# Zehong-Ma/MagCache

Measured on NVIDIA H100. Metric: denoising_steps_per_sec, higher is better.
Workload: dtype bf16

## Files before the change

magcache_b200/build.py:

```python
import os
import shutil
import subprocess
import sys

HERE = os.path.dirname(os.path.abspath(__file__))
CSRC = os.path.join(HERE, "csrc")
LIB = os.path.join(HERE, "libmagcache_b200.so")
SOURCES = ["controller.cu", "cache_kernels.cu", "rowwise_kernels.cu", "gemm_wgmma.cu", "attn_wgmma.cu", "head_wgmma.cu", "p2p.cu", "dit_forward.cu", "nccl_gather.cu"]
NVCC_FLAGS = ["-gencode", "arch=compute_90a,code=sm_90a", "-O3", "-std=c++17", "-lineinfo", "-Xcompiler", "-fPIC",
              "-Xptxas", "-v", "--expt-relaxed-constexpr"]


def _nvcc():
    return shutil.which("nvcc") or "/usr/local/cuda/bin/nvcc"


def _stale():
    if not os.path.exists(LIB):
        return True
    t = os.path.getmtime(LIB)
    deps = [os.path.join(CSRC, f) for f in os.listdir(CSRC)] + [os.path.join(HERE, "..", "include", "magcache_b200.h"), __file__]
    return any(os.path.getmtime(d) > t for d in deps)


def build(force=False, verbose=False):
    if not force and not _stale():
        return LIB
    objs = []
    bdir = os.path.join(HERE, "build")
    os.makedirs(bdir, exist_ok=True)
    procs = []
    for src in SOURCES:
        obj = os.path.join(bdir, src.replace(".cu", ".o"))
        cmd = [_nvcc(), *NVCC_FLAGS, "-c", os.path.join(CSRC, src), "-o", obj]
        procs.append((src, subprocess.Popen(cmd, stdout=subprocess.PIPE, stderr=subprocess.STDOUT, text=True)))
        objs.append(obj)
    log = []
    for src, p in procs:
        out, _ = p.communicate()
        log.append(f"==== {src}\n{out}")
        if p.returncode != 0:
            sys.stderr.write(out)
            raise RuntimeError(f"nvcc failed on {src}")
    with open(os.path.join(bdir, "ptxas.log"), "w") as f:
        f.write("\n".join(log))
    if verbose:
        print("\n".join(log))
    serialised = [line.strip() for line in "\n".join(log).splitlines() if "C7510" in line]
    if serialised:
        raise RuntimeError("ptxas serialised wgmma (C7510); no kernel that issues wgmma may contain a function call such as "
                           "device printf (see MC_DEVICE_DIAG in csrc/ptx.cuh). Full log: build/ptxas.log\n" +
                           "\n".join(serialised[:8]))
    cmd = [_nvcc(), "-shared", "-o", LIB, *objs, "-gencode", "arch=compute_90a,code=sm_90a", "-cudart", "static", "-ldl"]
    subprocess.check_call(cmd)
    return LIB


if __name__ == "__main__":
    print(build(force="--force" in sys.argv, verbose="-v" in sys.argv))
```

magcache_b200/csrc/attn_wgmma.cu:

```cuda
#include <cstdlib>

#include "common.cuh"
#include "ptx.cuh"
#include "tma_host.cuh"

#ifndef MC_ATTN_EMU_DEFAULT
#define MC_ATTN_EMU_DEFAULT 0
#endif

namespace mc {

constexpr int kHD = 128;
constexpr int kLongMinLk = 1024;

struct AttnParams {
  int Lq, Lk, heads;
  int q_blocks, full_units, tail_units, tail_split;
  float* part_o;
  float2* part_ml;
  float scale_log2;
  __nv_bfloat16* out;
  int64_t ldo;
  int tile_rot;
  const uint32_t* seg_flags;
// ... 13 lines not shown
  if (c < p.full_units) {
    unit = c, w.split = 0, w.nsplit = 1, w.tail_unit = 0;
  } else {
    c -= p.full_units;
    w.tail_unit = c / p.tail_split;
    w.split = c - w.tail_unit * p.tail_split;
    w.nsplit = p.tail_split;
    unit = p.full_units + w.tail_unit;
  }
  w.head = unit / p.q_blocks;
  w.q_block = unit - w.head * p.q_blocks;
  return w;
}

template <uint32_t EMU_MASK>
__device__ __forceinline__ float exp2_sel(float x, int group) {
  return ((EMU_MASK >> (group & 7)) & 1u) ? ptx::ex2_emul(x) : ptx::ex2_approx(x);
}

__device__ __forceinline__ void wait_segments(const AttnParams& p, int row0, int rows) {
  if (p.seg_flags == nullptr) return;
  const uint32_t want = *reinterpret_cast<const volatile uint32_t*>(p.seg_epoch);
  const int last = min(row0 + rows, p.Lk) - 1;
  const int s0 = row0 / p.seg_rows, s1 = last / p.seg_rows;
  for (int s = s0; s <= s1; ++s) {
    const uint32_t* f = p.seg_flags + s;
    const long long t0 = clock64();
    for (;;) {
      uint32_t v;
      asm volatile("ld.acquire.sys.global.u32 %0, [%1];" : "=r"(v) : "l"(f) : "memory");
      if (static_cast<int32_t>(v - want) >= 0) break;
      __nanosleep(100);
      if (clock64() - t0 > MC_MBAR_TIMEOUT_CYCLES) {
        MC_DIAG("attention: key segment %d never arrived (flag %u, epoch %u)\n", s, v, want);
        __trap();
      }
    }
  }
  asm volatile("fence.proxy.async;" ::: "memory");
}

namespace ak {
constexpr int kBQ = 128;
constexpr int kQBytes = kBQ * kHD * 2;
constexpr int kThreads = 384;
constexpr int kProducerRegs = 24, kConsumerRegs = 240;
template <int BKV>
struct Layout {
  static constexpr int kKBytes = BKV * kHD * 2;
  static constexpr int kVBytes = BKV * kHD * 2;
  static constexpr int kOffK = kQBytes;
  static constexpr int kOffV = kOffK + 2 * kKBytes;
  static constexpr int kOffBar = kOffV + 2 * kVBytes;
  static constexpr int kSmem = kOffBar + 128;
};
}

template <int BKV, uint32_t EMU_MASK>
__global__ void __launch_bounds__(ak::kThreads, 1)
    attn_kernel(const __grid_constant__ CUtensorMap tmap_q, const __grid_constant__ CUtensorMap tmap_k,
                const __grid_constant__ CUtensorMap tmap_v, const AttnParams p) {
  using namespace ak;
  using L = Layout<BKV>;
  extern __shared__ __align__(1024) uint8_t smem[];
  uint64_t* bars = reinterpret_cast<uint64_t*>(smem + L::kOffBar);
  uint64_t* q_full = bars + 0;
  uint64_t* k_full = bars + 1;
  uint64_t* k_empty = bars + 3;
  uint64_t* v_full = bars + 5;
  uint64_t* v_empty = bars + 7;

  const int warp = threadIdx.x >> 5, lane = threadIdx.x & 31;
  const WorkItem wi = work_item(p);
  const int q0 = wi.q_block * kBQ;
  const int head = wi.head;
  const int total_tiles = (p.Lk + BKV - 1) / BKV;
  const int per_split = (total_tiles + wi.nsplit - 1) / wi.nsplit;
  const int t0 = wi.split * per_split;
  const int n_tiles = min(per_split, total_tiles - t0);
  auto tile_of = [&](int j) {
    int t = p.tile_rot + t0 + j;
    return t >= total_tiles ? t - total_tiles : t;
  };

  if (threadIdx.x == 0) {
    if ((ptx::smem_u32(smem) & 1023u) != 0) {
      MC_DIAG("attn_kernel: dynamic smem base not 1024-aligned\n");
      __trap();
    }
    ptx::prefetch_tmap(&tmap_q);
    ptx::prefetch_tmap(&tmap_k);
    ptx::prefetch_tmap(&tmap_v);
    ptx::mbar_init(q_full, 1);
    for (int s = 0; s < 2; ++s) {
      ptx::mbar_init(&k_full[s], 1);
      ptx::mbar_init(&k_empty[s], 8);
      ptx::mbar_init(&v_full[s], 1);
      ptx::mbar_init(&v_empty[s], 8);
    }
    ptx::fence_mbar_init();
  }
  __syncthreads();

  if (warp < 4) {
    ptx::setmaxnreg_dec<kProducerRegs>();
    if (warp == 0) {
      if (ptx::elect_one()) {
        ptx::mbar_expect_tx(q_full, kQBytes);
        ptx::tma_load_2d(smem, &tmap_q, q_full, head * kHD, q0);
        ptx::tma_load_2d(smem + kQBytes / 2, &tmap_q, q_full, head * kHD + 64, q0);
      }
      __syncwarp();
      for (int j = 0; j < n_tiles; ++j) {
        const int s = j & 1;
        const uint32_t ph = (j >> 1) & 1;
        const int kv0 = tile_of(j) * BKV;
        if (p.seg_flags != nullptr) {
          if (lane == 0) wait_segments(p, kv0, BKV);
          __syncwarp();
        }
        ptx::mbar_wait(&k_empty[s], ph ^ 1);
        if (ptx::elect_one()) {
          ptx::mbar_expect_tx(&k_full[s], L::kKBytes);
          ptx::tma_load_2d(smem + L::kOffK + s * L::kKBytes, &tmap_k, &k_full[s], head * kHD, kv0);
          ptx::tma_load_2d(smem + L::kOffK + s * L::kKBytes + L::kKBytes / 2, &tmap_k, &k_full[s], head * kHD + 64, kv0);
        }
        __syncwarp();
        ptx::mbar_wait(&v_empty[s], ph ^ 1);
        if (ptx::elect_one()) {
          ptx::mbar_expect_tx(&v_full[s], L::kVBytes);
          ptx::tma_load_2d(smem + L::kOffV + s * L::kVBytes, &tmap_v, &v_full[s], head * kHD, kv0);
          ptx::tma_load_2d(smem + L::kOffV + s * L::kVBytes + L::kVBytes / 2, &tmap_v, &v_full[s], head * kHD + 64, kv0);
        }
        __syncwarp();
      }
    }
  } else {
    ptx::setmaxnreg_inc<kConsumerRegs>();
    const int wg = (warp >> 2) - 1;
    const int r = wg * 64 + (warp & 3) * 16 + (lane >> 2);
    const int cq = 2 * (lane & 3);
    const uint32_t q_base = ptx::smem_u32(smem) + wg * (64 * 128);
    const uint32_t k_base = ptx::smem_u32(smem + L::kOffK), v_base = ptx::smem_u32(smem + L::kOffV);
    int j_ragged = -1;
    if (p.Lk % BKV != 0) {
      int jr = total_tiles - 1 - p.tile_rot - t0;
      if (jr < 0) jr += total_tiles;
      if (jr < n_tiles) j_ragged = jr;
    }
    float o[kHD / 2];
#pragma unroll
    for (int i = 0; i < kHD / 2; ++i) o[i] = 0.f;
    float m0 = -INFINITY, m1 = -INFINITY, l0 = 0.f, l1 = 0.f;
    ptx::mbar_wait(q_full, 0);

    constexpr uint32_t kTurnThreads = 256;
    const uint32_t bar_own = 1 + wg, bar_other = 2 - wg;
    auto turn_begin = [&] { ptx::named_bar_sync(bar_own, kTurnThreads); };
    auto turn_end = [&] { ptx::named_bar_arrive(bar_other, kTurnThreads); };
    if (wg == 0) ptx::named_bar_arrive(bar_own, kTurnThreads);

    float sc[BKV / 2];
    uint32_t pa[BKV / 16][4];
    const int valid = p.Lk - (total_tiles - 1) * BKV;
    auto issue_s = [&](int j) {
      const int s = j & 1;
      ptx::wgmma_fence();
#pragma unroll
      for (int kk = 0; kk < kHD / 16; ++kk) {
        const uint64_t da = ptx::gmma_desc_sw128_kmajor(q_base + (kk >> 2) * (kQBytes / 2)) + 2 * (kk & 3);
        const uint64_t db = ptx::gmma_desc_sw128_kmajor(k_base + s * L::kKBytes + (kk >> 2) * (L::kKBytes / 2)) + 2 * (kk & 3);
        if constexpr (BKV == 128) {
          ptx::wgmma_m64n128k16_ss(sc, da, db, kk != 0 ? 1u : 0u);
        } else {
          ptx::wgmma_m64n64k16_ss(sc, da, db, kk != 0 ? 1u : 0u);
        }
      }
      ptx::wgmma_commit();
    };
    auto issue_pv = [&](int j) {
      const int s = j & 1;
      ptx::fence_regs(o);
      ptx::wgmma_fence();
      const uint64_t dv = ptx::gmma_desc_sw128_mnmajor(v_base + s * L::kVBytes, BKV * 128);
#pragma unroll
      for (int kk = 0; kk < BKV / 16; ++kk)
        ptx::wgmma_m64n128k16_rs_tb(o, pa[kk], dv + static_cast<uint64_t>(kk * (2048 / 16)), 1u);
      ptx::wgmma_commit();
    };
    auto softmax = [&](int j, float& f0, float& f1) {
      ptx::fence_regs(sc);
      __syncwarp();
      if (lane == 0) ptx::mbar_arrive(&k_empty[j & 1]);
      if (j == j_ragged) {
#pragma unroll
        for (int i = 0; i < BKV / 8; ++i)
#pragma unroll
          for (int e = 0; e < 4; ++e)
            if (8 * i + cq + (e & 1) >= valid) sc[4 * i + e] = -INFINITY;
      }
      float mx0 = -INFINITY, mx1 = -INFINITY;
#pragma unroll
      for (int i = 0; i < BKV / 8; ++i) {
        mx0 = fmaxf(mx0, fmaxf(sc[4 * i], sc[4 * i + 1]));
        mx1 = fmaxf(mx1, fmaxf(sc[4 * i + 2], sc[4 * i + 3]));
      }
#pragma unroll
      for (int off = 1; off <= 2; off <<= 1) {
        mx0 = fmaxf(mx0, __shfl_xor_sync(0xffffffffu, mx0, off));
        mx1 = fmaxf(mx1, __shfl_xor_sync(0xffffffffu, mx1, off));
      }
      const float mn0 = fmaxf(m0, mx0 * p.scale_log2), mn1 = fmaxf(m1, mx1 * p.scale_log2);
      f0 = ptx::ex2_approx(m0 - mn0), f1 = ptx::ex2_approx(m1 - mn1);
      m0 = mn0, m1 = mn1;
      l0 *= f0, l1 *= f1;
#pragma unroll
      for (int i = 0; i < BKV / 8; ++i) {
        sc[4 * i] = exp2_sel<EMU_MASK>(fmaf(sc[4 * i], p.scale_log2, -m0), i);
        sc[4 * i + 1] = exp2_sel<EMU_MASK>(fmaf(sc[4 * i + 1], p.scale_log2, -m0), i);
        sc[4 * i + 2] = exp2_sel<EMU_MASK>(fmaf(sc[4 * i + 2], p.scale_log2, -m1), i);
        sc[4 * i + 3] = exp2_sel<EMU_MASK>(fmaf(sc[4 * i + 3], p.scale_log2, -m1), i);
        l0 += sc[4 * i] + sc[4 * i + 1];
        l1 += sc[4 * i + 2] + sc[4 * i + 3];
      }
    };
    auto pack_p = [&] {
#pragma unroll
      for (int i = 0; i < BKV / 8; ++i) {
        pa[i >> 1][(i & 1) * 2] = pack_bf16x2(sc[4 * i], sc[4 * i + 1]);
        pa[i >> 1][(i & 1) * 2 + 1] = pack_bf16x2(sc[4 * i + 2], sc[4 * i + 3]);
      }
    };
    auto release_v = [&](int j) {
      ptx::fence_regs(o);
      __syncwarp();
      if (lane == 0) ptx::mbar_arrive(&v_empty[j & 1]);
    };
    auto rescale_o = [&](float f0, float f1) {
#pragma unroll
      for (int i = 0; i < kHD / 8; ++i) {
        o[4 * i] *= f0, o[4 * i + 1] *= f0;
        o[4 * i + 2] *= f1, o[4 * i + 3] *= f1;
      }
    };
    for (int j = 0; j < n_tiles; ++j) {
      ptx::mbar_wait(&k_full[j & 1], (j >> 1) & 1);
      turn_begin();
      issue_s(j);
      turn_end();
      ptx::wgmma_wait<0>();
      float f0, f1;
      softmax(j, f0, f1);
      rescale_o(f0, f1);
      pack_p();
      ptx::mbar_wait(&v_full[j & 1], (j >> 1) & 1);
      turn_begin();
      issue_pv(j);
      if (wg == 0 || j + 1 < n_tiles) turn_end();
      ptx::wgmma_wait<0>();
      release_v(j);
    }

#pragma unroll
    for (int off = 1; off <= 2; off <<= 1) {
      l0 += __shfl_xor_sync(0xffffffffu, l0, off);
      l1 += __shfl_xor_sync(0xffffffffu, l1, off);
    }
    const bool partial = wi.nsplit > 1;
#pragma unroll
    for (int h = 0; h < 2; ++h) {
      const float inv_l = 1.0f / (h ? l1 : l0);
      const int rt = r + 8 * h;
      const int row = q0 + rt;
      if (row >= p.Lq) continue;
      if (partial) {
        const int64_t prow = (static_cast<int64_t>(wi.split) * p.tail_units + wi.tail_unit) * kBQ + rt;
        if ((lane & 3) == 0) p.part_ml[prow] = make_float2(h ? m1 : m0, h ? l1 : l0);
        float* dst = p.part_o + prow * kHD + cq;
#pragma unroll
        for (int i = 0; i < kHD / 8; ++i)
          *reinterpret_cast<float2*>(dst + 8 * i) = make_float2(o[4 * i + 2 * h] * inv_l, o[4 * i + 2 * h + 1] * inv_l);
      } else {
        __nv_bfloat16* dst = p.out + static_cast<int64_t>(row) * p.ldo + head * kHD + cq;
#pragma unroll
        for (int i = 0; i < kHD / 8; ++i)
          *reinterpret_cast<uint32_t*>(dst + 8 * i) = pack_bf16x2(o[4 * i + 2 * h] * inv_l, o[4 * i + 2 * h + 1] * inv_l);
      }
    }
  }
}

__global__ void __launch_bounds__(256) attn_combine_kernel(const float* __restrict__ part_o, const float2* __restrict__ part_ml, int nsplit,
                                                           int tail_units, int full_units, int q_blocks, int rows_per_cta, int Lq,
                                                           __nv_bfloat16* __restrict__ out, int64_t ldo) {
  constexpr int kGroups = kHD / 8;
  const int64_t total = static_cast<int64_t>(tail_units) * rows_per_cta * kGroups;
  const int64_t split_stride = static_cast<int64_t>(tail_units) * rows_per_cta;
  for (int64_t i = static_cast<int64_t>(blockIdx.x) * blockDim.x + threadIdx.x; i < total; i += static_cast<int64_t>(gridDim.x) * blockDim.x) {
    const int64_t prow = i / kGroups;
    const int g = static_cast<int>(i - prow * kGroups);
    const int tu = static_cast<int>(prow / rows_per_cta), r = static_cast<int>(prow - static_cast<int64_t>(tu) * rows_per_cta);
    const int unit = full_units + tu;
    const int head = unit / q_blocks, row = (unit - head * q_blocks) * rows_per_cta + r;
    if (row >= Lq) continue;
    float mmax = -INFINITY;
    for (int s = 0; s < nsplit; ++s) mmax = fmaxf(mmax, part_ml[s * split_stride + prow].x);
    float acc[8] = {0.f, 0.f, 0.f, 0.f, 0.f, 0.f, 0.f, 0.f};
    float wsum = 0.f;
    for (int s = 0; s < nsplit; ++s) {
      const float2 ml = part_ml[s * split_stride + prow];
      const float w = ml.y * ptx::ex2_approx(ml.x - mmax);
      wsum += w;
      float v[8];
      ptx::ld_nc_v8_f32(part_o + (s * split_stride + prow) * kHD + g * 8, v);
#pragma unroll
      for (int j = 0; j < 8; ++j) acc[j] = fmaf(w, v[j], acc[j]);
    }
    const float inv = 1.0f / wsum;
#pragma unroll
    for (int j = 0; j < 8; ++j) acc[j] *= inv;
    *reinterpret_cast<uint4*>(out + static_cast<int64_t>(row) * ldo + head * kHD + g * 8) = pack_bf16x8(acc);
  }
}

struct AttnPlan {
  bool long_kernel;
  int q_blocks, kv_tile, total_tiles, rows_per_cta;
  int full_units, tail_units, tail_split;
  size_t ws_bytes;
  int grid() const { return full_units + tail_units * tail_split; }
};

static int env_int(const char* name, int lo, int hi, int dflt) {
  const char* e = getenv(name);
  if (!e || !*e) return dflt;
  const int v = atoi(e);
  return (v < lo || v > hi) ? dflt : v;
}

static AttnPlan plan_attention(int Lq, int Lk, int heads, bool need_long = false) {
  AttnPlan pl;
  const int forced_splits = env_int("MC_ATTN_SPLITS", 1, 16, 0);
  const int kernel_sel = env_int("MC_ATTN_KERNEL", 0, 2, 0);
  pl.long_kernel = need_long || kernel_sel == 2 || (kernel_sel == 0 && Lk >= kLongMinLk);
  pl.rows_per_cta = ak::kBQ;
  pl.kv_tile = pl.long_kernel ? 128 : 64;
  pl.q_blocks = (Lq + pl.rows_per_cta - 1) / pl.rows_per_cta;
  pl.total_tiles = (Lk + pl.kv_tile - 1) / pl.kv_tile;
  const int64_t units = static_cast<int64_t>(pl.q_blocks) * heads;
  const int slots = num_sms();
  const int min_tiles_per_split = pl.long_kernel ? 4 : 8;
  int full = static_cast<int>(units), tail = 0, split = 1;
  if (forced_splits > 0) {
    if (forced_splits > 1) full = 0, tail = static_cast<int>(units), split = forced_splits;
  } else {
    const int rem = static_cast<int>(units % slots);
    const int by_tiles = pl.total_tiles / min_tiles_per_split;
    int f = rem > 0 ? slots / rem : 1;
    if (f > 8) f = 8;
    if (f > by_tiles) f = by_tiles;
    if (f >= 2) full = static_cast<int>(units) - rem, tail = rem, split = f;
  }
  if (split > pl.total_tiles) split = pl.total_tiles;
  if (split > 1) {
    const int per = (pl.total_tiles + split - 1) / split;
    split = (pl.total_tiles + per - 1) / per;
  }
  if (split <= 1) full = static_cast<int>(units), tail = 0, split = 1;
  pl.full_units = full, pl.tail_units = tail, pl.tail_split = split;
  pl.ws_bytes = tail > 0 ? static_cast<size_t>(split) * tail * pl.rows_per_cta * (kHD * sizeof(float) + sizeof(float2)) : 0;
  return pl;
}

}

extern "C" int32_t mc_attn_workspace_bytes(int32_t Lq, int32_t Lk, int32_t heads, int64_t* bytes_out) {
  MC_CHECK_ARG(bytes_out != nullptr && Lq >= 1 && Lk >= 1 && heads >= 1, "mc_attn_workspace_bytes: bad arguments");
  const size_t a = mc::plan_attention(Lq, Lk, heads, false).ws_bytes, b = mc::plan_attention(Lq, Lk, heads, true).ws_bytes;
  *bytes_out = static_cast<int64_t>(a > b ? a : b);
  return MC_OK;
}

extern "C" int32_t mc_attn_fwd_ex(const void* q, int64_t ldq, const void* k, int64_t ldk, const void* v, int64_t ldv, void* out,
                                  int64_t ldo, int32_t Lq, int32_t Lk, int32_t heads, float scale, void* workspace,
                                  int64_t workspace_bytes, int32_t first_key_row, const uint32_t* seg_flags, const uint32_t* seg_epoch,
                                  int32_t seg_rows, void* stream) {
  MC_CHECK_ARG(q && k && v && out, "mc_attn_fwd: null pointer");
  MC_CHECK_ARG(Lq >= 1 && Lk >= 1 && heads >= 1, "mc_attn_fwd: Lq=%d Lk=%d heads=%d", Lq, Lk, heads);
  const int64_t width = static_cast<int64_t>(heads) * mc::kHD;
  MC_CHECK_ARG(ldq >= width && ldk >= width && ldo >= width && ldv >= width, "mc_attn_fwd: leading dimensions too small");
  MC_CHECK_ARG(ldq % 8 == 0 && ldk % 8 == 0 && ldv % 8 == 0 && ldo % 8 == 0, "mc_attn_fwd: leading dimensions must be multiples of 8");
  MC_CHECK_ARG(mc::aligned16(q) && mc::aligned16(k) && mc::aligned16(v) && mc::aligned16(out), "mc_attn_fwd: pointers must be 16-byte aligned");
  MC_CHECK_ARG(first_key_row >= 0 && first_key_row < Lk, "mc_attn_fwd: first_key_row=%d outside [0, %d)", first_key_row, Lk);
  MC_CHECK_ARG(seg_flags == nullptr || (seg_rows >= 1 && seg_epoch != nullptr), "mc_attn_fwd: seg_rows=%d / null epoch", seg_rows);
  const mc::AttnPlan pl = mc::plan_attention(Lq, Lk, heads, first_key_row != 0 || seg_flags != nullptr);
  MC_CHECK_ARG(static_cast<int64_t>(pl.q_blocks) * heads * 8 < INT32_MAX, "mc_attn_fwd: grid too large");
  if (pl.tail_units > 0) {
    MC_CHECK_ARG(workspace != nullptr && workspace_bytes >= static_cast<int64_t>(pl.ws_bytes) && (reinterpret_cast<uintptr_t>(workspace) & 31u) == 0,
                 "mc_attn_fwd: split-KV needs a 32-byte aligned workspace of %lld bytes (mc_attn_workspace_bytes), got %lld",
                 static_cast<long long>(pl.ws_bytes), static_cast<long long>(workspace_bytes));
  }
  const int q_box = mc::ak::kBQ;
  CUtensorMap tq, tk, tv;
  int32_t rc = mc::make_tmap_bf16_2d(&tq, q, static_cast<uint64_t>(Lq), static_cast<uint64_t>(width), static_cast<uint64_t>(ldq), q_box, 64);
  if (rc) return rc;
  rc = mc::make_tmap_bf16_2d(&tk, k, static_cast<uint64_t>(Lk), static_cast<uint64_t>(width), static_cast<uint64_t>(ldk), pl.kv_tile, 64);
  if (rc) return rc;
  rc = mc::make_tmap_bf16_2d(&tv, v, static_cast<uint64_t>(Lk), static_cast<uint64_t>(width), static_cast<uint64_t>(ldv), pl.kv_tile, 64);
  if (rc) return rc;

  float* part_o = static_cast<float*>(workspace);
  const size_t part_rows = static_cast<size_t>(pl.tail_split) * pl.tail_units * pl.rows_per_cta;
  float2* part_ml = pl.tail_units > 0 ? reinterpret_cast<float2*>(part_o + part_rows * mc::kHD) : nullptr;
  mc::AttnParams p{};
// ... 49 lines not shown
```

magcache_b200/csrc/gemm_wgmma.cu:

```cuda
#include <cstdlib>

#include "common.cuh"
#include "ptx.cuh"
#include "tma_host.cuh"

namespace mc {

TmapCacheEntry* tmap_cache() {
  static TmapCacheEntry table[kTmapCacheSize] = {};
  return table;
}
std::mutex& tmap_cache_mutex() {
  static std::mutex m;
  return m;
}

constexpr int kBM = 128, kBK = 64, kStages = 4;
constexpr int kTileABytes = kBM * kBK * 2;
constexpr int kStagePad = 33;
constexpr int kEpiWarps = 8;
constexpr int kStagingBytes = kEpiWarps * 32 * kStagePad * 4;
constexpr int kGemmThreads = 128 + 32 * kEpiWarps;
constexpr int kProducerRegs = 40, kConsumerRegs = 232;
template <int BN>
struct GemmTile {
  static constexpr int kTileBBytes = BN * kBK * 2;
  static constexpr int kStageBytes = kTileABytes + kTileBBytes;
  static constexpr int kOffStaging = kStages * kStageBytes;
  static constexpr int kOffBars = kOffStaging + kStagingBytes;
  static constexpr int kSmem = kOffBars + 128;
};

struct GemmParams {
  int M, N, K;
  const float* bias;
  void* out;
  int64_t ldo;
  const float* gate;
};

template <int EPI>
__device__ __forceinline__ void epilogue_patch(const GemmParams& p, const float* stage, int row0, int col0, int lane) {
  const int rows = min(32, p.M - row0);
  if (rows <= 0) return;
  const int col = col0 + lane;
  const bool col_ok = col < p.N;

  if (EPI == MC_EPI_BIAS_GATE_RESID) {
    const float b = (p.bias && col_ok) ? p.bias[col] : 0.f;
    const float g = (p.gate && col_ok) ? p.gate[col] : 1.f;
    float* xcol = static_cast<float*>(p.out) + static_cast<int64_t>(row0) * p.ldo + col;
    float xv[32];
#pragma unroll
    for (int r = 0; r < 32; ++r) xv[r] = (col_ok && r < rows) ? xcol[static_cast<int64_t>(r) * p.ldo] : 0.f;
#pragma unroll
    for (int r = 0; r < 32; ++r) {
      const float y = round_bf16(stage[r * kStagePad + lane] + b);
      xv[r] = __fadd_rn(xv[r], __fmul_rn(y, g));
    }
#pragma unroll
    for (int r = 0; r < 32; ++r)
      if (col_ok && r < rows) xcol[static_cast<int64_t>(r) * p.ldo] = xv[r];
    return;
  }

  if (EPI == MC_EPI_BIAS_F32) {
    const float b = (p.bias && col_ok) ? p.bias[col] : 0.f;
    float* ocol = static_cast<float*>(p.out) + static_cast<int64_t>(row0) * p.ldo + col;
#pragma unroll
    for (int r = 0; r < 32; ++r)
      if (col_ok && r < rows) ocol[static_cast<int64_t>(r) * p.ldo] = stage[r * kStagePad + lane] + b;
    return;
  }

  const int half = lane >> 4, cp = (lane & 15) * 2;
  const int c0 = col0 + cp;
  float b0 = 0.f, b1 = 0.f;
  if (EPI != MC_EPI_ROWBIAS_BF16 && p.bias) {
    if (c0 < p.N) b0 = p.bias[c0];
    if (c0 + 1 < p.N) b1 = p.bias[c0 + 1];
  }
  float g0 = 1.f, g1 = 1.f;
  if (EPI == MC_EPI_BIAS_GATE_RESID_BF16 && p.gate) {
    if (c0 < p.N) g0 = p.gate[c0];
    if (c0 + 1 < p.N) g1 = p.gate[c0 + 1];
  }
  __nv_bfloat16* obase = static_cast<__nv_bfloat16*>(p.out) + static_cast<int64_t>(row0 + half) * p.ldo + c0;
  const float* sbase = stage + half * kStagePad + cp;
  const float* rbias = (EPI == MC_EPI_ROWBIAS_BF16 && p.bias) ? p.bias + row0 + half : nullptr;

  if (rows == 32 && col0 + 32 <= p.N && (p.ldo & 1) == 0) {
    uint32_t w[16];
#pragma unroll
    for (int i = 0; i < 16; ++i) {
      float v0 = sbase[2 * i * kStagePad], v1 = sbase[2 * i * kStagePad + 1];
      if (EPI == MC_EPI_ROWBIAS_BF16) {
        const float rb = rbias ? rbias[2 * i] : 0.f;
        v0 += rb;
        v1 += rb;
      } else {
        v0 += b0;
        v1 += b1;
      }
      if (EPI == MC_EPI_BIAS_GELU_BF16) {
        v0 = gelu_tanh(round_bf16(v0));
        v1 = gelu_tanh(round_bf16(v1));
      }
      if (EPI == MC_EPI_BIAS_GELU_ERF_BF16) {
        v0 = gelu_erf(round_bf16(v0));
        v1 = gelu_erf(round_bf16(v1));
      }
      if (EPI == MC_EPI_BIAS_SILU_BF16) {
        v0 = silu_f(round_bf16(v0));
        v1 = silu_f(round_bf16(v1));
      }
      if (EPI == MC_EPI_BIAS_GATE_RESID_BF16) {
        const uint32_t old = *reinterpret_cast<const uint32_t*>(obase + static_cast<int64_t>(2 * i) * p.ldo);
        v0 = bf16_lo(old) + round_bf16(g0 * round_bf16(v0));
        v1 = bf16_hi(old) + round_bf16(g1 * round_bf16(v1));
      }
      w[i] = pack_bf16x2(v0, v1);
    }
#pragma unroll
    for (int i = 0; i < 16; ++i) *reinterpret_cast<uint32_t*>(obase + static_cast<int64_t>(2 * i) * p.ldo) = w[i];
    return;
  }

  const bool pair_ok = (c0 + 1 < p.N) && ((p.ldo & 1) == 0);
  for (int i = 0; i < 16; ++i) {
    const int r = 2 * i + half;
    if (r >= rows) continue;
    float v0 = sbase[2 * i * kStagePad], v1 = sbase[2 * i * kStagePad + 1];
    if (EPI == MC_EPI_ROWBIAS_BF16) {
      const float rb = rbias ? rbias[2 * i] : 0.f;
      v0 += rb;
      v1 += rb;
    } else {
      v0 += b0;
      v1 += b1;
    }
    if (EPI == MC_EPI_BIAS_GELU_BF16) {
      v0 = gelu_tanh(round_bf16(v0));
      v1 = gelu_tanh(round_bf16(v1));
    }
    if (EPI == MC_EPI_BIAS_GELU_ERF_BF16) {
      v0 = gelu_erf(round_bf16(v0));
      v1 = gelu_erf(round_bf16(v1));
    }
    if (EPI == MC_EPI_BIAS_SILU_BF16) {
      v0 = silu_f(round_bf16(v0));
      v1 = silu_f(round_bf16(v1));
    }
    __nv_bfloat16* o = obase + static_cast<int64_t>(2 * i) * p.ldo;
    if (EPI == MC_EPI_BIAS_GATE_RESID_BF16) {
      if (c0 < p.N) v0 = __bfloat162float(o[0]) + round_bf16(g0 * round_bf16(v0));
      if (c0 + 1 < p.N) v1 = __bfloat162float(o[1]) + round_bf16(g1 * round_bf16(v1));
    }
    if (pair_ok) {
      *reinterpret_cast<uint32_t*>(o) = pack_bf16x2(v0, v1);
    } else {
      if (c0 < p.N) o[0] = __float2bfloat16_rn(v0);
      if (c0 + 1 < p.N) o[1] = __float2bfloat16_rn(v1);
    }
  }
}

template <int EPI, int kBN>
__global__ void __launch_bounds__(kGemmThreads, 1)
    gemm_bf16_kernel(const __grid_constant__ CUtensorMap tmap_a, const __grid_constant__ CUtensorMap tmap_b, const GemmParams p) {
  using T = GemmTile<kBN>;
  constexpr int kStageBytes = T::kStageBytes, kOffStaging = T::kOffStaging, kOffBars = T::kOffBars;
  extern __shared__ __align__(1024) uint8_t smem[];
  float* staging = reinterpret_cast<float*>(smem + kOffStaging);
  uint64_t* full_bar = reinterpret_cast<uint64_t*>(smem + kOffBars);
  uint64_t* empty_bar = full_bar + kStages;

  const int warp = threadIdx.x >> 5, lane = threadIdx.x & 31;
  const int m_tiles = (p.M + kBM - 1) / kBM, n_tiles = (p.N + kBN - 1) / kBN;
  const int total_tiles = m_tiles * n_tiles;
  const int num_kb = (p.K + kBK - 1) / kBK;

  if (threadIdx.x == 0) {
    if ((ptx::smem_u32(smem) & 1023u) != 0) {
      MC_DIAG("gemm_bf16_kernel: dynamic smem base not 1024-aligned\n");
      __trap();
    }
    ptx::prefetch_tmap(&tmap_a);
    ptx::prefetch_tmap(&tmap_b);
    for (int s = 0; s < kStages; ++s) {
      ptx::mbar_init(&full_bar[s], 1);
      ptx::mbar_init(&empty_bar[s], kEpiWarps);
    }
    ptx::fence_mbar_init();
  }
  __syncthreads();

  if (warp < 4) {
    ptx::setmaxnreg_dec<kProducerRegs>();
    if (warp == 0) {
      uint32_t it = 0;
      for (int tile = blockIdx.x; tile < total_tiles; tile += gridDim.x) {
        const int m0 = (tile / n_tiles) * kBM, n0 = (tile % n_tiles) * kBN;
        for (int kb = 0; kb < num_kb; ++kb, ++it) {
          const int s = it % kStages;
          const uint32_t ph = (it / kStages) & 1;
          ptx::mbar_wait(&empty_bar[s], ph ^ 1);
          if (ptx::elect_one()) {
            uint8_t* sa = smem + s * kStageBytes;
            ptx::mbar_expect_tx(&full_bar[s], kStageBytes);
            ptx::tma_load_2d(sa, &tmap_a, &full_bar[s], kb * kBK, m0);
            ptx::tma_load_2d(sa + kTileABytes, &tmap_b, &full_bar[s], kb * kBK, n0);
          }
          __syncwarp();
        }
      }
    }
  } else {
    ptx::setmaxnreg_inc<kConsumerRegs>();
    const int wg = (warp >> 2) - 1;
    const int wq = warp & 3;
    float acc[kBN / 2];
    uint32_t it = 0;
    for (int tile = blockIdx.x; tile < total_tiles; tile += gridDim.x) {
      const int m0 = (tile / n_tiles) * kBM, n0 = (tile % n_tiles) * kBN;
      int prev_s = -1;
      for (int kb = 0; kb < num_kb; ++kb, ++it) {
        const int s = it % kStages;
        const uint32_t ph = (it / kStages) & 1;
        ptx::mbar_wait(&full_bar[s], ph);
        const uint32_t sa = ptx::smem_u32(smem + s * kStageBytes);
        const uint64_t da = ptx::gmma_desc_sw128_kmajor(sa + wg * (64 * 128));
        const uint64_t db = ptx::gmma_desc_sw128_kmajor(sa + kTileABytes);
        ptx::wgmma_fence();
#pragma unroll
        for (int k = 0; k < kBK / 16; ++k) {
          if constexpr (kBN == 256) {
            ptx::wgmma_m64n256k16_ss(acc, da + 2 * k, db + 2 * k, (kb | k) != 0 ? 1u : 0u);
          } else {
            ptx::wgmma_m64n128k16_ss(acc, da + 2 * k, db + 2 * k, (kb | k) != 0 ? 1u : 0u);
          }
        }
        ptx::wgmma_commit();
        ptx::wgmma_wait<1>();
        ptx::fence_regs(acc);
        if (prev_s >= 0 && lane == 0) ptx::mbar_arrive(&empty_bar[prev_s]);
        prev_s = s;
      }
      ptx::wgmma_wait<0>();
      ptx::fence_regs(acc);
      if (lane == 0) ptx::mbar_arrive(&empty_bar[prev_s]);

      const int pr = wq >> 1;
      const int row0 = m0 + wg * 64 + pr * 32;
      const int r_lo = (wq & 1) * 16 + (lane >> 2);
#pragma unroll
      for (int c = 0; c < kBN / 32; ++c) {
        float* patch = staging + (4 * wg + 2 * pr + (c & 1)) * 32 * kStagePad;
        asm volatile("bar.sync %0, 64;" ::"r"(1 + 2 * wg + pr) : "memory");
#pragma unroll
        for (int q = 0; q < 4; ++q) {
          const int i = 4 * c + q;
          const int col = 8 * q + 2 * (lane & 3);
          patch[r_lo * kStagePad + col] = acc[4 * i + 0];
          patch[r_lo * kStagePad + col + 1] = acc[4 * i + 1];
          patch[(r_lo + 8) * kStagePad + col] = acc[4 * i + 2];
          patch[(r_lo + 8) * kStagePad + col + 1] = acc[4 * i + 3];
        }
        asm volatile("bar.sync %0, 64;" ::"r"(1 + 2 * wg + pr) : "memory");
        if ((wq & 1) == (c & 1)) epilogue_patch<EPI>(p, patch, row0, n0 + c * 32, lane);
      }
    }
  }
}

template <int EPI, int BN>
static int32_t launch_gemm_bn(const CUtensorMap& ta, const CUtensorMap& tb, const GemmParams& p, cudaStream_t s) {
  static PerDeviceOnce once;
  const int32_t rc = set_max_smem_once(gemm_bf16_kernel<EPI, BN>, GemmTile<BN>::kSmem, once, "cudaFuncSetAttribute(gemm smem)");
  if (rc) return rc;
  const int m_tiles = (p.M + kBM - 1) / kBM, n_tiles = (p.N + BN - 1) / BN;
  const int total = m_tiles * n_tiles;
  const int grid = total < num_sms() ? total : num_sms();
  gemm_bf16_kernel<EPI, BN><<<grid, kGemmThreads, GemmTile<BN>::kSmem, s>>>(ta, tb, p);
  MC_CHECK_LAUNCH("gemm_bf16_kernel launch");
  return MC_OK;
}

static int pick_bn(int M, int N) {
  const char* e = getenv("MC_GEMM_BN");
  if (e && *e) {
    const int v = atoi(e);
    if (v == 128 || v == 256) return v;
  }
  const int64_t sms = num_sms(), m_tiles = (M + kBM - 1) / kBM;
  const int64_t t256 = m_tiles * ((N + 255) / 256), t128 = m_tiles * ((N + 127) / 128);
  const int64_t cost256 = ((t256 + sms - 1) / sms) * 100, cost128 = ((t128 + sms - 1) / sms) * 62;
  return cost128 * 100 <= cost256 * 92 ? 128 : 256;
}

}

extern "C" int32_t mc_gemm_bf16(const void* A, int64_t lda, const void* B, int64_t ldb, int32_t M, int32_t N, int32_t K,
                                const float* bias, int32_t epilogue, void* out, int64_t ldo, const float* gate, void* stream) {
  MC_CHECK_ARG(A && B && out, "mc_gemm_bf16: null pointer");
  MC_CHECK_ARG(M >= 1 && N >= 1 && K >= 8, "mc_gemm_bf16: M=%d N=%d K=%d", M, N, K);
  MC_CHECK_ARG(K % 8 == 0 && lda % 8 == 0 && ldb % 8 == 0 && lda >= K && ldb >= K, "mc_gemm_bf16: K/lda/ldb must be multiples of 8 (16-byte TMA pitch)");
  MC_CHECK_ARG(mc::aligned16(A) && mc::aligned16(B) && mc::aligned16(out), "mc_gemm_bf16: A/B/out must be 16-byte aligned");
  MC_CHECK_ARG(ldo >= N, "mc_gemm_bf16: ldo=%lld < N=%d", static_cast<long long>(ldo), N);
  CUtensorMap ta, tb;
  int32_t rc = mc::make_tmap_bf16_2d(&ta, A, static_cast<uint64_t>(M), static_cast<uint64_t>(K), static_cast<uint64_t>(lda), mc::kBM, mc::kBK);
  if (rc) return rc;
  const int bn = mc::pick_bn(M, N);
  rc = mc::make_tmap_bf16_2d(&tb, B, static_cast<uint64_t>(N), static_cast<uint64_t>(K), static_cast<uint64_t>(ldb), bn, mc::kBK);
  if (rc) return rc;
  mc::GemmParams p{M, N, K, bias, out, ldo, gate};
  cudaStream_t s = static_cast<cudaStream_t>(stream);
#define MC_GEMM_CASE(E) \
  case E: return bn == 128 ? mc::launch_gemm_bn<E, 128>(ta, tb, p, s) : mc::launch_gemm_bn<E, 256>(ta, tb, p, s)
  switch (epilogue) {
    MC_GEMM_CASE(MC_EPI_BIAS_BF16);
    MC_GEMM_CASE(MC_EPI_BIAS_GELU_BF16);
    MC_GEMM_CASE(MC_EPI_BIAS_GATE_RESID);
    MC_GEMM_CASE(MC_EPI_ROWBIAS_BF16);
    MC_GEMM_CASE(MC_EPI_BIAS_F32);
    MC_GEMM_CASE(MC_EPI_BIAS_GELU_ERF_BF16);
    MC_GEMM_CASE(MC_EPI_BIAS_GATE_RESID_BF16);
    MC_GEMM_CASE(MC_EPI_BIAS_SILU_BF16);
#undef MC_GEMM_CASE
    default:
      mc::set_error("mc_gemm_bf16: unknown epilogue %d", epilogue);
      return MC_ERR_INVALID;
  }
}
```

magcache_b200/csrc/ptx.cuh:

```cuda
#pragma once
#include <cstdint>
#include <cuda_runtime.h>

namespace ptx {

__device__ __forceinline__ uint32_t smem_u32(const void* p) {
  return static_cast<uint32_t>(__cvta_generic_to_shared(p));
}

__device__ __forceinline__ void mbar_init(uint64_t* bar, uint32_t count) {
  asm volatile("mbarrier.init.shared::cta.b64 [%0], %1;" ::"r"(smem_u32(bar)), "r"(count) : "memory");
}
__device__ __forceinline__ void fence_mbar_init() {
  asm volatile("fence.mbarrier_init.release.cluster;" ::: "memory");
}
__device__ __forceinline__ void mbar_expect_tx(uint64_t* bar, uint32_t bytes) {
  asm volatile("mbarrier.arrive.expect_tx.shared::cta.b64 _, [%0], %1;" ::"r"(smem_u32(bar)), "r"(bytes) : "memory");
}
__device__ __forceinline__ void mbar_arrive(uint64_t* bar) {
  asm volatile("mbarrier.arrive.shared::cta.b64 _, [%0];" ::"r"(smem_u32(bar)) : "memory");
}
__device__ __forceinline__ bool mbar_try_wait(uint64_t* bar, uint32_t parity) {
  uint32_t ok;
  asm volatile(
      "{\n"
      ".reg .pred p;\n"
      "mbarrier.try_wait.parity.shared::cta.b64 p, [%1], %2;\n"
      "selp.u32 %0, 1, 0, p;\n"
      "}\n"
      : "=r"(ok)
      : "r"(smem_u32(bar)), "r"(parity)
      : "memory");
  return ok != 0;
}
#ifndef MC_DEVICE_DIAG
#define MC_DEVICE_DIAG 0
#endif
#if MC_DEVICE_DIAG
#define MC_DIAG(...) printf(__VA_ARGS__)
#else
#define MC_DIAG(...) ((void)0)
#endif

#ifndef MC_MBAR_TIMEOUT_CYCLES
#define MC_MBAR_TIMEOUT_CYCLES (4000000000ll)
#endif
__device__ __forceinline__ void mbar_wait(uint64_t* bar, uint32_t parity) {
  if (mbar_try_wait(bar, parity)) return;
  const long long t0 = clock64();
  while (!mbar_try_wait(bar, parity)) {
    if (clock64() - t0 > MC_MBAR_TIMEOUT_CYCLES) {
      MC_DIAG("mbar_wait timeout: block (%d,%d,%d) thread %d bar smem+%u parity %u\n", blockIdx.x, blockIdx.y, blockIdx.z,
              threadIdx.x, smem_u32(bar), parity);
      __trap();
    }
  }
}

__device__ __forceinline__ void named_bar_sync(uint32_t id, uint32_t count) {
  asm volatile("bar.sync %0, %1;" ::"r"(id), "r"(count) : "memory");
}
__device__ __forceinline__ void named_bar_arrive(uint32_t id, uint32_t count) {
  asm volatile("bar.arrive %0, %1;" ::"r"(id), "r"(count) : "memory");
}

__device__ __forceinline__ bool elect_one() {
  uint32_t pred;
  asm volatile(
      "{\n"
      ".reg .pred P;\n"
      "elect.sync _|P, 0xffffffff;\n"
      "selp.u32 %0, 1, 0, P;\n"
      "}\n"
      : "=r"(pred));
  return pred != 0;
}

__device__ __forceinline__ void fence_proxy_async_smem() {
  asm volatile("fence.proxy.async.shared::cta;" ::: "memory");
}

__device__ __forceinline__ void prefetch_tmap(const void* tmap) {
  asm volatile("prefetch.tensormap [%0];" ::"l"(reinterpret_cast<uint64_t>(tmap)) : "memory");
}
__device__ __forceinline__ void tma_load_2d(void* smem_dst, const void* tmap, uint64_t* bar, int32_t c0, int32_t c1) {
  asm volatile(
      "cp.async.bulk.tensor.2d.shared::cluster.global.mbarrier::complete_tx::bytes [%0], [%1, {%3, %4}], [%2];"
      ::"r"(smem_u32(smem_dst)), "l"(reinterpret_cast<uint64_t>(tmap)), "r"(smem_u32(bar)), "r"(c0), "r"(c1)
      : "memory");
}

__device__ __forceinline__ void bulk_load_1d(void* smem_dst, const void* gmem_src, uint32_t bytes, uint64_t* bar) {
  asm volatile("cp.async.bulk.shared::cluster.global.mbarrier::complete_tx::bytes [%0], [%1], %2, [%3];" ::"r"(smem_u32(smem_dst)),
               "l"(reinterpret_cast<uint64_t>(gmem_src)), "r"(bytes), "r"(smem_u32(bar))
               : "memory");
}

__device__ __forceinline__ uint64_t gmma_desc_sw128_kmajor(uint32_t smem_addr) {
  uint64_t d = 0;
  d |= static_cast<uint64_t>((smem_addr & 0x3FFFFu) >> 4);
  d |= static_cast<uint64_t>(1) << 16;
  d |= static_cast<uint64_t>(1024 >> 4) << 32;
  d |= static_cast<uint64_t>(1) << 62;
  return d;
}
__device__ __forceinline__ uint64_t gmma_desc_sw128_mnmajor(uint32_t smem_addr, uint32_t lbo_bytes, uint32_t sbo_bytes = 1024) {
  uint64_t d = 0;
  d |= static_cast<uint64_t>((smem_addr & 0x3FFFFu) >> 4);
  d |= static_cast<uint64_t>((lbo_bytes >> 4) & 0x3FFFu) << 16;
  d |= static_cast<uint64_t>((sbo_bytes >> 4) & 0x3FFFu) << 32;
  d |= static_cast<uint64_t>(1) << 62;
  return d;
}
__device__ __forceinline__ void wgmma_fence() { asm volatile("wgmma.fence.sync.aligned;" ::: "memory"); }
__device__ __forceinline__ void wgmma_commit() { asm volatile("wgmma.commit_group.sync.aligned;" ::: "memory"); }
template <int N>
__device__ __forceinline__ void wgmma_wait() {
  asm volatile("wgmma.wait_group.sync.aligned %0;" ::"n"(N) : "memory");
}
template <int N>
__device__ __forceinline__ void fence_regs(float (&d)[N]) {
#pragma unroll
  for (int i = 0; i < N; ++i) asm volatile("" : "+f"(d[i])::"memory");
}

__device__ __forceinline__ void wgmma_m64n64k16_ss(float (&d)[32], uint64_t adesc, uint64_t bdesc, uint32_t accumulate) {
  asm volatile(
      "{\n"
      ".reg .pred p;\n"
      "setp.ne.b32 p, %34, 0;\n"
      "wgmma.mma_async.sync.aligned.m64n64k16.f32.bf16.bf16 "
      "{%0, %1, %2, %3, %4, %5, %6, %7, %8, %9, %10, %11, %12, %13, %14, %15, %16, %17, %18, %19, %20, %21, %22, %23, %24, %25, %26, %27, %28, %29, %30, %31}, "
      "%32, %33, p, 1, 1, 0, 0;\n"
      "}\n"
      : "+f"(d[0]), "+f"(d[1]), "+f"(d[2]), "+f"(d[3]), "+f"(d[4]), "+f"(d[5]), "+f"(d[6]), "+f"(d[7]), "+f"(d[8]), "+f"(d[9]), "+f"(d[10]), "+f"(d[11]), "+f"(d[12]), "+f"(d[13]), "+f"(d[14]), "+f"(d[15]), "+f"(d[16]), "+f"(d[17]), "+f"(d[18]), "+f"(d[19]), "+f"(d[20]), "+f"(d[21]), "+f"(d[22]), "+f"(d[23]), "+f"(d[24]), "+f"(d[25]), "+f"(d[26]), "+f"(d[27]), "+f"(d[28]), "+f"(d[29]), "+f"(d[30]), "+f"(d[31])
      : "l"(adesc), "l"(bdesc), "r"(accumulate));
}
__device__ __forceinline__ void wgmma_m64n128k16_ss(float (&d)[64], uint64_t adesc, uint64_t bdesc, uint32_t accumulate) {
  asm volatile(
      "{\n"
      ".reg .pred p;\n"
      "setp.ne.b32 p, %66, 0;\n"
      "wgmma.mma_async.sync.aligned.m64n128k16.f32.bf16.bf16 "
      "{%0, %1, %2, %3, %4, %5, %6, %7, %8, %9, %10, %11, %12, %13, %14, %15, %16, %17, %18, %19, %20, %21, %22, %23, %24, %25, %26, %27, %28, %29, %30, %31, %32, %33, %34, %35, %36, %37, %38, %39, %40, %41, %42, %43, %44, %45, %46, %47, %48, %49, %50, %51, %52, %53, %54, %55, %56, %57, %58, %59, %60, %61, %62, %63}, "
      "%64, %65, p, 1, 1, 0, 0;\n"
      "}\n"
      : "+f"(d[0]), "+f"(d[1]), "+f"(d[2]), "+f"(d[3]), "+f"(d[4]), "+f"(d[5]), "+f"(d[6]), "+f"(d[7]), "+f"(d[8]), "+f"(d[9]), "+f"(d[10]), "+f"(d[11]), "+f"(d[12]), "+f"(d[13]), "+f"(d[14]), "+f"(d[15]), "+f"(d[16]), "+f"(d[17]), "+f"(d[18]), "+f"(d[19]), "+f"(d[20]), "+f"(d[21]), "+f"(d[22]), "+f"(d[23]), "+f"(d[24]), "+f"(d[25]), "+f"(d[26]), "+f"(d[27]), "+f"(d[28]), "+f"(d[29]), "+f"(d[30]), "+f"(d[31]), "+f"(d[32]), "+f"(d[33]), "+f"(d[34]), "+f"(d[35]), "+f"(d[36]), "+f"(d[37]), "+f"(d[38]), "+f"(d[39]), "+f"(d[40]), "+f"(d[41]), "+f"(d[42]), "+f"(d[43]), "+f"(d[44]), "+f"(d[45]), "+f"(d[46]), "+f"(d[47]), "+f"(d[48]), "+f"(d[49]), "+f"(d[50]), "+f"(d[51]), "+f"(d[52]), "+f"(d[53]), "+f"(d[54]), "+f"(d[55]), "+f"(d[56]), "+f"(d[57]), "+f"(d[58]), "+f"(d[59]), "+f"(d[60]), "+f"(d[61]), "+f"(d[62]), "+f"(d[63])
      : "l"(adesc), "l"(bdesc), "r"(accumulate));
}
__device__ __forceinline__ void wgmma_m64n256k16_ss(float (&d)[128], uint64_t adesc, uint64_t bdesc, uint32_t accumulate) {
  asm volatile(
      "{\n"
      ".reg .pred p;\n"
      "setp.ne.b32 p, %130, 0;\n"
      "wgmma.mma_async.sync.aligned.m64n256k16.f32.bf16.bf16 "
      "{%0, %1, %2, %3, %4, %5, %6, %7, %8, %9, %10, %11, %12, %13, %14, %15, %16, %17, %18, %19, %20, %21, %22, %23, %24, %25, %26, %27, %28, %29, %30, %31, %32, %33, %34, %35, %36, %37, %38, %39, %40, %41, %42, %43, %44, %45, %46, %47, %48, %49, %50, %51, %52, %53, %54, %55, %56, %57, %58, %59, %60, %61, %62, %63, %64, %65, %66, %67, %68, %69, %70, %71, %72, %73, %74, %75, %76, %77, %78, %79, %80, %81, %82, %83, %84, %85, %86, %87, %88, %89, %90, %91, %92, %93, %94, %95, %96, %97, %98, %99, %100, %101, %102, %103, %104, %105, %106, %107, %108, %109, %110, %111, %112, %113, %114, %115, %116, %117, %118, %119, %120, %121, %122, %123, %124, %125, %126, %127}, "
      "%128, %129, p, 1, 1, 0, 0;\n"
      "}\n"
      : "+f"(d[0]), "+f"(d[1]), "+f"(d[2]), "+f"(d[3]), "+f"(d[4]), "+f"(d[5]), "+f"(d[6]), "+f"(d[7]), "+f"(d[8]), "+f"(d[9]), "+f"(d[10]), "+f"(d[11]), "+f"(d[12]), "+f"(d[13]), "+f"(d[14]), "+f"(d[15]), "+f"(d[16]), "+f"(d[17]), "+f"(d[18]), "+f"(d[19]), "+f"(d[20]), "+f"(d[21]), "+f"(d[22]), "+f"(d[23]), "+f"(d[24]), "+f"(d[25]), "+f"(d[26]), "+f"(d[27]), "+f"(d[28]), "+f"(d[29]), "+f"(d[30]), "+f"(d[31]), "+f"(d[32]), "+f"(d[33]), "+f"(d[34]), "+f"(d[35]), "+f"(d[36]), "+f"(d[37]), "+f"(d[38]), "+f"(d[39]), "+f"(d[40]), "+f"(d[41]), "+f"(d[42]), "+f"(d[43]), "+f"(d[44]), "+f"(d[45]), "+f"(d[46]), "+f"(d[47]), "+f"(d[48]), "+f"(d[49]), "+f"(d[50]), "+f"(d[51]), "+f"(d[52]), "+f"(d[53]), "+f"(d[54]), "+f"(d[55]), "+f"(d[56]), "+f"(d[57]), "+f"(d[58]), "+f"(d[59]), "+f"(d[60]), "+f"(d[61]), "+f"(d[62]), "+f"(d[63]), "+f"(d[64]), "+f"(d[65]), "+f"(d[66]), "+f"(d[67]), "+f"(d[68]), "+f"(d[69]), "+f"(d[70]), "+f"(d[71]), "+f"(d[72]), "+f"(d[73]), "+f"(d[74]), "+f"(d[75]), "+f"(d[76]), "+f"(d[77]), "+f"(d[78]), "+f"(d[79]), "+f"(d[80]), "+f"(d[81]), "+f"(d[82]), "+f"(d[83]), "+f"(d[84]), "+f"(d[85]), "+f"(d[86]), "+f"(d[87]), "+f"(d[88]), "+f"(d[89]), "+f"(d[90]), "+f"(d[91]), "+f"(d[92]), "+f"(d[93]), "+f"(d[94]), "+f"(d[95]), "+f"(d[96]), "+f"(d[97]), "+f"(d[98]), "+f"(d[99]), "+f"(d[100]), "+f"(d[101]), "+f"(d[102]), "+f"(d[103]), "+f"(d[104]), "+f"(d[105]), "+f"(d[106]), "+f"(d[107]), "+f"(d[108]), "+f"(d[109]), "+f"(d[110]), "+f"(d[111]), "+f"(d[112]), "+f"(d[113]), "+f"(d[114]), "+f"(d[115]), "+f"(d[116]), "+f"(d[117]), "+f"(d[118]), "+f"(d[119]), "+f"(d[120]), "+f"(d[121]), "+f"(d[122]), "+f"(d[123]), "+f"(d[124]), "+f"(d[125]), "+f"(d[126]), "+f"(d[127])
      : "l"(adesc), "l"(bdesc), "r"(accumulate));
}
__device__ __forceinline__ void wgmma_m64n128k16_rs_tb(float (&d)[64], const uint32_t (&a)[4], uint64_t bdesc, uint32_t accumulate) {
  asm volatile(
      "{\n"
      ".reg .pred p;\n"
      "setp.ne.b32 p, %69, 0;\n"
      "wgmma.mma_async.sync.aligned.m64n128k16.f32.bf16.bf16 "
      "{%0, %1, %2, %3, %4, %5, %6, %7, %8, %9, %10, %11, %12, %13, %14, %15, %16, %17, %18, %19, %20, %21, %22, %23, %24, %25, %26, %27, %28, %29, %30, %31, %32, %33, %34, %35, %36, %37, %38, %39, %40, %41, %42, %43, %44, %45, %46, %47, %48, %49, %50, %51, %52, %53, %54, %55, %56, %57, %58, %59, %60, %61, %62, %63}, "
      "{%64, %65, %66, %67}, %68, p, 1, 1, 1;\n"
      "}\n"
      : "+f"(d[0]), "+f"(d[1]), "+f"(d[2]), "+f"(d[3]), "+f"(d[4]), "+f"(d[5]), "+f"(d[6]), "+f"(d[7]), "+f"(d[8]), "+f"(d[9]), "+f"(d[10]), "+f"(d[11]), "+f"(d[12]), "+f"(d[13]), "+f"(d[14]), "+f"(d[15]), "+f"(d[16]), "+f"(d[17]), "+f"(d[18]), "+f"(d[19]), "+f"(d[20]), "+f"(d[21]), "+f"(d[22]), "+f"(d[23]), "+f"(d[24]), "+f"(d[25]), "+f"(d[26]), "+f"(d[27]), "+f"(d[28]), "+f"(d[29]), "+f"(d[30]), "+f"(d[31]), "+f"(d[32]), "+f"(d[33]), "+f"(d[34]), "+f"(d[35]), "+f"(d[36]), "+f"(d[37]), "+f"(d[38]), "+f"(d[39]), "+f"(d[40]), "+f"(d[41]), "+f"(d[42]), "+f"(d[43]), "+f"(d[44]), "+f"(d[45]), "+f"(d[46]), "+f"(d[47]), "+f"(d[48]), "+f"(d[49]), "+f"(d[50]), "+f"(d[51]), "+f"(d[52]), "+f"(d[53]), "+f"(d[54]), "+f"(d[55]), "+f"(d[56]), "+f"(d[57]), "+f"(d[58]), "+f"(d[59]), "+f"(d[60]), "+f"(d[61]), "+f"(d[62]), "+f"(d[63])
      : "r"(a[0]), "r"(a[1]), "r"(a[2]), "r"(a[3]), "l"(bdesc), "r"(accumulate));
}


template <int N>
__device__ __forceinline__ void setmaxnreg_inc() {
  asm volatile("setmaxnreg.inc.sync.aligned.u32 %0;" ::"n"(N));
}
template <int N>
__device__ __forceinline__ void setmaxnreg_dec() {
  asm volatile("setmaxnreg.dec.sync.aligned.u32 %0;" ::"n"(N));
}

__device__ __forceinline__ float ex2_approx(float x) {
  float y;
  asm("ex2.approx.ftz.f32 %0, %1;" : "=f"(y) : "f"(x));
  return y;
}
__device__ __forceinline__ float ex2_emul(float x) {
  const float kMagic = 12582912.0f;
  x = fmaxf(x, -126.0f);
  const float t = __fadd_rd(x, kMagic);
  const float f = x - __fadd_rn(t, -kMagic);
  float p = __fmaf_rn(0.077119089663028717041015625f, f, 0.227564394474029541015625f);
  p = __fmaf_rn(p, f, 0.695146143436431884765625f);
  p = __fmaf_rn(p, f, 1.0f);
  return __int_as_float(__float_as_int(p) + (__float_as_int(t) << 23));
}
__device__ __forceinline__ uint4 ld_nc_v4(const void* p) {
  uint4 r;
  asm volatile("ld.global.nc.L1::no_allocate.v4.u32 {%0, %1, %2, %3}, [%4];" : "=r"(r.x), "=r"(r.y), "=r"(r.z), "=r"(r.w) : "l"(p));
  return r;
}
__device__ __forceinline__ void st_na_v4(void* p, const uint4& v) {
  asm volatile("st.global.L1::no_allocate.v4.u32 [%0], {%1, %2, %3, %4};" ::"l"(p), "r"(v.x), "r"(v.y), "r"(v.z), "r"(v.w) : "memory");
}

__device__ __forceinline__ void ld_nc_v8_f32(const float* p, float (&f)[8]) {
  asm volatile("ld.global.nc.L1::no_allocate.v4.f32 {%0, %1, %2, %3}, [%4];" : "=f"(f[0]), "=f"(f[1]), "=f"(f[2]), "=f"(f[3]) : "l"(p));
// ... 12 lines not shown
```

Measured before the change: 1.187.

## Software-pipeline attention S and PV wgmmas and reduce GEMM epilogue register pressure

Restructures the attention consumer loop so the QK^T wgmma for tile j and the PV wgmma for tile j-1 are issued together, with softmax of tile j overlapping the in-flight PV. The point is to hide tensor-core latency behind softmax work. The GEMM gate-residual epilogue now processes rows in halves to cut live registers, and total_tiles is passed in from the host. The build now fails on register spills or C7512 serialization, and the mbarrier waits in attention record a timeout flag and trap after the loop instead of trapping inside it. The pipelined loop keeps more accumulator registers live, which risks spills.

```diff
diff --git a/magcache_b200/build.py b/magcache_b200/build.py
--- a/magcache_b200/build.py
+++ b/magcache_b200/build.py
@@ -1,4 +1,5 @@
 import os
+import re
 import shutil
 import subprocess
 import sys
@@ -9,6 +10,7 @@
 SOURCES = ["controller.cu", "cache_kernels.cu", "rowwise_kernels.cu", "gemm_wgmma.cu", "attn_wgmma.cu", "head_wgmma.cu", "p2p.cu", "dit_forward.cu", "nccl_gather.cu"]
 NVCC_FLAGS = ["-gencode", "arch=compute_90a,code=sm_90a", "-O3", "-std=c++17", "-lineinfo", "-Xcompiler", "-fPIC",
               "-Xptxas", "-v", "--expt-relaxed-constexpr"]
+NO_SPILL_KERNELS = ("attn_kernel", "gemm_bf16_kernel")
 
 
 def _nvcc():
@@ -21,6 +23,27 @@
     t = os.path.getmtime(LIB)
     deps = [os.path.join(CSRC, f) for f in os.listdir(CSRC)] + [os.path.join(HERE, "..", "include", "magcache_b200.h"), __file__]
     return any(os.path.getmtime(d) > t for d in deps)
+
+
+def _check_ptxas(log):
+    serialised = [line.strip() for line in log.splitlines() if "C7510" in line or "C7512" in line]
+    if serialised:
+        raise RuntimeError("ptxas serialised wgmma (C7510: the kernel contains a function call such as device printf, see "
+                           "MC_DEVICE_DIAG in csrc/ptx.cuh; C7512: not enough registers). Full log: build/ptxas.log\n" +
+                           "\n".join(serialised[:8]))
+    spills, fn = [], None
+    for line in log.splitlines():
+        m = re.search(r"Function properties for (\S+)", line)
+        if m:
+            fn = m.group(1)
+            continue
+        m = re.search(r"(\d+) bytes spill stores", line)
+        if m and fn is not None:
+            if int(m.group(1)) > 0 and any(k in fn for k in NO_SPILL_KERNELS):
+                spills.append(f"{fn}: {line.strip()}")
+            fn = None
+    if spills:
+        raise RuntimeError("ptxas spilled registers in a kernel that issues wgmma. Full log: build/ptxas.log\n" + "\n".join(spills))
 
 
 def build(force=False, verbose=False):
@@ -46,11 +69,7 @@
         f.write("\n".join(log))
     if verbose:
         print("\n".join(log))
-    serialised = [line.strip() for line in "\n".join(log).splitlines() if "C7510" in line]
-    if serialised:
-        raise RuntimeError("ptxas serialised wgmma (C7510); no kernel that issues wgmma may contain a function call such as "
-                           "device printf (see MC_DEVICE_DIAG in csrc/ptx.cuh). Full log: build/ptxas.log\n" +
-                           "\n".join(serialised[:8]))
+    _check_ptxas("\n".join(log))
     cmd = [_nvcc(), "-shared", "-o", LIB, *objs, "-gencode", "arch=compute_90a,code=sm_90a", "-cudart", "static", "-ldl"]
     subprocess.check_call(cmd)
     return LIB
diff --git a/magcache_b200/csrc/attn_wgmma.cu b/magcache_b200/csrc/attn_wgmma.cu
--- a/magcache_b200/csrc/attn_wgmma.cu
+++ b/magcache_b200/csrc/attn_wgmma.cu
@@ -189,7 +189,8 @@
 #pragma unroll
     for (int i = 0; i < kHD / 2; ++i) o[i] = 0.f;
     float m0 = -INFINITY, m1 = -INFINITY, l0 = 0.f, l1 = 0.f;
-    ptx::mbar_wait(q_full, 0);
+    bool timed_out = false;
+    ptx::mbar_wait_or_flag(q_full, 0, timed_out);
 
     constexpr uint32_t kTurnThreads = 256;
     const uint32_t bar_own = 1 + wg, bar_other = 2 - wg;
@@ -280,23 +281,42 @@
         o[4 * i + 2] *= f1, o[4 * i + 3] *= f1;
       }
     };
-    for (int j = 0; j < n_tiles; ++j) {
-      ptx::mbar_wait(&k_full[j & 1], (j >> 1) & 1);
+    {
+      ptx::mbar_wait_or_flag(&k_full[0], 0, timed_out);
       turn_begin();
-      issue_s(j);
+      issue_s(0);
       turn_end();
       ptx::wgmma_wait<0>();
       float f0, f1;
-      softmax(j, f0, f1);
+      softmax(0, f0, f1);
       rescale_o(f0, f1);
       pack_p();
-      ptx::mbar_wait(&v_full[j & 1], (j >> 1) & 1);
+    }
+    for (int j = 1; j < n_tiles; ++j) {
+      ptx::mbar_wait_or_flag(&k_full[j & 1], (j >> 1) & 1, timed_out);
+      ptx::mbar_wait_or_flag(&v_full[(j - 1) & 1], ((j - 1) >> 1) & 1, timed_out);
+      turn_begin();
+      issue_s(j);
+      issue_pv(j - 1);
+      turn_end();
+      ptx::wgmma_wait<1>();
+      float f0, f1;
+      softmax(j, f0, f1);
+      ptx::wgmma_wait<0>();
+      release_v(j - 1);
+      rescale_o(f0, f1);
+      pack_p();
+    }
+    {
+      const int j = n_tiles - 1;
+      ptx::mbar_wait_or_flag(&v_full[j & 1], (j >> 1) & 1, timed_out);
       turn_begin();
       issue_pv(j);
-      if (wg == 0 || j + 1 < n_tiles) turn_end();
+      if (wg == 0) turn_end();
       ptx::wgmma_wait<0>();
       release_v(j);
     }
+    if (timed_out) __trap();
 
 #pragma unroll
     for (int off = 1; off <= 2; off <<= 1) {
diff --git a/magcache_b200/csrc/gemm_wgmma.cu b/magcache_b200/csrc/gemm_wgmma.cu
--- a/magcache_b200/csrc/gemm_wgmma.cu
+++ b/magcache_b200/csrc/gemm_wgmma.cu
@@ -37,6 +37,7 @@
   void* out;
   int64_t ldo;
   const float* gate;
+  int total_tiles;
 };
 
 template <int EPI>
@@ -50,17 +51,20 @@
     const float b = (p.bias && col_ok) ? p.bias[col] : 0.f;
     const float g = (p.gate && col_ok) ? p.gate[col] : 1.f;
     float* xcol = static_cast<float*>(p.out) + static_cast<int64_t>(row0) * p.ldo + col;
-    float xv[32];
-#pragma unroll
-    for (int r = 0; r < 32; ++r) xv[r] = (col_ok && r < rows) ? xcol[static_cast<int64_t>(r) * p.ldo] : 0.f;
-#pragma unroll
-    for (int r = 0; r < 32; ++r) {
-      const float y = round_bf16(stage[r * kStagePad + lane] + b);
-      xv[r] = __fadd_rn(xv[r], __fmul_rn(y, g));
-    }
-#pragma unroll
-    for (int r = 0; r < 32; ++r)
-      if (col_ok && r < rows) xcol[static_cast<int64_t>(r) * p.ldo] = xv[r];
+#pragma unroll
+    for (int h = 0; h < 32; h += 16) {
+      float xv[16];
+#pragma unroll
+      for (int r = 0; r < 16; ++r) xv[r] = (col_ok && h + r < rows) ? xcol[static_cast<int64_t>(h + r) * p.ldo] : 0.f;
+#pragma unroll
+      for (int r = 0; r < 16; ++r) {
+        const float y = round_bf16(stage[(h + r) * kStagePad + lane] + b);
+        xv[r] = __fadd_rn(xv[r], __fmul_rn(y, g));
+      }
+#pragma unroll
+      for (int r = 0; r < 16; ++r)
+        if (col_ok && h + r < rows) xcol[static_cast<int64_t>(h + r) * p.ldo] = xv[r];
+    }
     return;
   }
 
@@ -176,8 +180,8 @@
   uint64_t* empty_bar = full_bar + kStages;
 
   const int warp = threadIdx.x >> 5, lane = threadIdx.x & 31;
-  const int m_tiles = (p.M + kBM - 1) / kBM, n_tiles = (p.N + kBN - 1) / kBN;
-  const int total_tiles = m_tiles * n_tiles;
+  const int n_tiles = (p.N + kBN - 1) / kBN;
+  const int total_tiles = p.total_tiles;
   const int num_kb = (p.K + kBK - 1) / kBK;
 
   if (threadIdx.x == 0) {
@@ -274,12 +278,13 @@
 }
 
 template <int EPI, int BN>
-static int32_t launch_gemm_bn(const CUtensorMap& ta, const CUtensorMap& tb, const GemmParams& p, cudaStream_t s) {
+static int32_t launch_gemm_bn(const CUtensorMap& ta, const CUtensorMap& tb, GemmParams p, cudaStream_t s) {
   static PerDeviceOnce once;
   const int32_t rc = set_max_smem_once(gemm_bf16_kernel<EPI, BN>, GemmTile<BN>::kSmem, once, "cudaFuncSetAttribute(gemm smem)");
   if (rc) return rc;
   const int m_tiles = (p.M + kBM - 1) / kBM, n_tiles = (p.N + BN - 1) / BN;
   const int total = m_tiles * n_tiles;
+  p.total_tiles = total;
   const int grid = total < num_sms() ? total : num_sms();
   gemm_bf16_kernel<EPI, BN><<<grid, kGemmThreads, GemmTile<BN>::kSmem, s>>>(ta, tb, p);
   MC_CHECK_LAUNCH("gemm_bf16_kernel launch");
@@ -313,7 +318,7 @@
   const int bn = mc::pick_bn(M, N);
   rc = mc::make_tmap_bf16_2d(&tb, B, static_cast<uint64_t>(N), static_cast<uint64_t>(K), static_cast<uint64_t>(ldb), bn, mc::kBK);
   if (rc) return rc;
-  mc::GemmParams p{M, N, K, bias, out, ldo, gate};
+  mc::GemmParams p{M, N, K, bias, out, ldo, gate, 0};
   cudaStream_t s = static_cast<cudaStream_t>(stream);
 #define MC_GEMM_CASE(E) \
   case E: return bn == 128 ? mc::launch_gemm_bn<E, 128>(ta, tb, p, s) : mc::launch_gemm_bn<E, 256>(ta, tb, p, s)
diff --git a/magcache_b200/csrc/ptx.cuh b/magcache_b200/csrc/ptx.cuh
--- a/magcache_b200/csrc/ptx.cuh
+++ b/magcache_b200/csrc/ptx.cuh
@@ -56,6 +56,18 @@
     }
   }
 }
+__device__ __forceinline__ void mbar_wait_or_flag(uint64_t* bar, uint32_t parity, bool& timed_out) {
+  if (timed_out || mbar_try_wait(bar, parity)) return;
+  const long long t0 = clock64();
+  while (!mbar_try_wait(bar, parity)) {
+    if (clock64() - t0 > MC_MBAR_TIMEOUT_CYCLES) {
+      MC_DIAG("mbar_wait timeout: block (%d,%d,%d) thread %d bar smem+%u parity %u\n", blockIdx.x, blockIdx.y, blockIdx.z,
+              threadIdx.x, smem_u32(bar), parity);
+      timed_out = true;
+      return;
+    }
+  }
+}
 
 __device__ __forceinline__ void named_bar_sync(uint32_t id, uint32_t count) {
   asm volatile("bar.sync %0, %1;" ::"r"(id), "r"(count) : "memory");
```

New measurement: 1.243 (median of 6 runs). +4.7%, better.
